# sulaimanvesal/PointCloudUDA

Hardware: AMD Instinct MI355X
Metric: adversarial train-step images/sec (seg+3 discr) at 256x256 (higher is better)
Workload: dtype bf16x3 MFMA (split-bf16, fp32 accumulate; fp32 storage); 1 GPU; MS-CMRSeg full UDA: UNet(PointNet head) + d1 + d2 + d4, 256x256x1, 4 classes; per_gpu_batch=32, global_batch=32, precision=bf16x3, parallelism=dp1, ranks_in_group=1, collective=none, streams=discriminators concurrent, d_target_forward=replayed from the adversarial pass of the same step, launch=eager (256 host cores for this rank)

## Files before the change

### pointcloududa_amd/csrc/conv_igemm.h

```cpp
#pragma once
#include "common.h"

#define IG_MAX_TAPS 36
#define IG_REC 40
#define IG_REC_BYTES 80
template <bool X3>
struct IgRec {
  static constexpr int BYTES = X3 ? 144 : 80;
};
#define IG_LO_OFF 64
static inline int ig_rec_bytes(bool x3) { return x3 ? 144 : 80; }

struct IgemmParams {
  pcuda_src x;
  int cin;
  int in_h, in_w;
  int in_shift;
  int in_row;
  pcuda_dst y;
  int cout;
  int out_w;
  int lh, lw;
  int oy_mul, oy_off, ox_mul, ox_off;
  int in_step;
  int ntaps, tg;
  signed char dy[IG_MAX_TAPS], dx[IG_MAX_TAPS];
  int dy_min, dx_min, ih_t, iw_t;
  const uint16_t* wpack;
  long long w_lo_off;
  int nchunks;
  const float* bias;
  float slope;
  int accumulate;
  float* stats;
  const float* red_a; long long red_sn, red_sc;
  const float* red_mean; const float* red_invstd;
  const float* mask_a; long long mask_sn; float mask_slope;
  int tw, th, tmagic;
  int tiles_x, tiles_y, n;
  int n_co_tiles;
  unsigned m_cot, m_tx, m_ty;
  int clamp;
  int dbg;
  unsigned long long* dbg_clk;
  int xq;
  int fold;
  int pair, lw2;
};

struct WgradParams {
  pcuda_src x;
  int cin;
  int in_h, in_w, in_shift, in_row;
  const float* dz; long long dz_sn, dz_sc;
  int cout, out_h, out_w;
  int stride;
  int ntaps;
  int ntaps_total, tap_groups;
  signed char dy[IG_MAX_TAPS], dx[IG_MAX_TAPS];
  int ih_t, iw_t;
  int dy_min, dx_min;
  int tw, th, tmagic;
  int tiles_x, tiles_y, n;
  int ksplit;
  int n_co_tiles, n_chunks;
  float* partial;
  int aligned4;
  int tw16;
  int xq;
  int dbg;
  int xcd_items;
  int xcd_slices;
};

#define WG_ZROW 272

struct PackParams {
  const float* w;
  uint16_t* out;
  int rec;
  int rows, red;
  long long s_row, s_red;
  int ntaps;
  signed char tap_src[IG_MAX_TAPS];
  int pair;
  int co_tile;
  int nchunks, n_co_tiles;
};

static inline int ig_co_blks(int rows) { return rows > 32 ? 2 : 1; }
#define IG_TY(pl, magic) (((pl) * (magic)) >> 16)
```

### pointcloududa_amd/csrc/conv_wgrad.hip

```cpp
#include "conv_igemm.h"
#include "conv_host.h"

__global__ __launch_bounds__(1024) void wgrad_reduce_kernel(const float* __restrict__ partial, long long numel,
                                                           int ksplit, float* __restrict__ dw, int accumulate,
                                                           int ntaps, const float* __restrict__ db_partial,
                                                           long long nb, float* __restrict__ db) {
  __shared__ float sh[16][64];
  const int lane = threadIdx.x & 63, kg = threadIdx.x >> 6, nkg = blockDim.x >> 6;
  const long long nblk_w = (numel + 63) / 64;
  long long blk = blockIdx.x;
  if (blk >= nblk_w) {
    blk -= nblk_w; partial = db_partial; numel = nb; dw = db; ntaps = 1;
  }
  const long long i = blk * 64 + lane;
  float s = 0.f;
  if (i < numel) {
    int k = kg;
    for (; k + 7 * nkg < ksplit; k += 8 * nkg) {
      float v[8];
#pragma unroll
      for (int u = 0; u < 8; ++u) v[u] = partial[(long long)(k + u * nkg) * numel + i];
#pragma unroll
      for (int u = 0; u < 8; ++u) s += v[u];
    }
    for (; k < ksplit; k += nkg) s += partial[(long long)k * numel + i];
  }
  sh[kg][lane] = s;
  __syncthreads();
  if (kg == 0 && i < numel) {
    float t = 0.f;
    for (int q = 0; q < nkg; ++q) t += sh[q][lane];
    long long o = i;
    if (ntaps > 1) {
      const long long cc = numel / ntaps;
      const long long tt = i / cc, r = i - tt * cc;
      o = r * ntaps + tt;
    }
    dw[o] = accumulate ? dw[o] + t : t;
  }
}

int launch_wgrad_reduce_taps(const float* partial, long long numel, int ksplit, float* dw, int accumulate, int ntaps,
                             const float* db_partial, long long nb, float* db, hipStream_t s) {
  int nkg = 1;
  while (nkg < 16 && nkg * 2 <= ksplit) nkg <<= 1;
  const unsigned nblk = (unsigned)cdiv(numel, 64) + (db ? (unsigned)cdiv(nb, 64) : 0u);
  hipLaunchKernelGGL(wgrad_reduce_kernel, dim3(nblk), dim3(64 * nkg), 0, s, partial, numel, ksplit, dw, accumulate, ntaps,
                     db_partial, db ? nb : 0, db);
  PCUDA_CHECK_LAUNCH("wgrad_reduce_kernel");
  return PCUDA_OK;
}
int launch_wgrad_reduce(const float* partial, long long numel, int ksplit, float* dw, int accumulate, const float* db_partial,
                        long long nb, float* db, hipStream_t s) {
  return launch_wgrad_reduce_taps(partial, numel, ksplit, dw, accumulate, 1, db_partial, nb, db, s);
}

struct ReduceJobs {
  int n;
  int first_block[PCUDA_REDUCE_MAX_JOBS + 1];
  pcuda_reduce_job j[PCUDA_REDUCE_MAX_JOBS];
};

__global__ __launch_bounds__(1024) void wgrad_reduce_batch_kernel(const ReduceJobs jobs) {
  __shared__ float sh[16][64];
  int lo = 0, hi = jobs.n - 1;
  while (lo < hi) {
    const int mid = (lo + hi + 1) >> 1;
    if (jobs.first_block[mid] <= (int)blockIdx.x) lo = mid; else hi = mid - 1;
  }
  const pcuda_reduce_job& jb = jobs.j[lo];
  const float* partial = jb.partial;
  long long numel = jb.numel;
  float* dw = jb.dw;
  int ntaps = jb.ntaps;
  const int ksplit = jb.ksplit, nkg = jb.nkg;
  const int lane = threadIdx.x & 63, kg = threadIdx.x >> 6;
  const long long nblk_w = (numel + 63) / 64;
  long long blk = (int)blockIdx.x - jobs.first_block[lo];
  if (blk >= nblk_w) { blk -= nblk_w; partial = jb.db_partial; numel = jb.nb; dw = jb.db; ntaps = 1; }
  const long long i = blk * 64 + lane;
  float s = 0.f;
  if (i < numel && kg < nkg) {
    int k = kg;
    for (; k + 7 * nkg < ksplit; k += 8 * nkg) {
      float v[8];
#pragma unroll
      for (int u = 0; u < 8; ++u) v[u] = partial[(long long)(k + u * nkg) * numel + i];
#pragma unroll
      for (int u = 0; u < 8; ++u) s += v[u];
    }
    for (; k < ksplit; k += nkg) s += partial[(long long)k * numel + i];
  }
  sh[kg][lane] = s;
  __syncthreads();
  if (kg == 0 && i < numel) {
    float t = 0.f;
    for (int q = 0; q < nkg; ++q) t += sh[q][lane];
    long long o = i;
    if (ntaps > 1) {
      const long long cc = numel / ntaps;
      const long long tt = i / cc, r = i - tt * cc;
      o = r * ntaps + tt;
    }
    dw[o] = jb.accumulate ? dw[o] + t : t;
  }
}

extern "C" int pcuda_wgrad_reduce_batch(const pcuda_reduce_job* host_jobs, int njobs, pcuda_stream_t s) {
  if (!host_jobs || njobs < 0) PCUDA_FAIL(PCUDA_E_BADARG, "wgrad_reduce_batch: bad arguments");
  int done = 0;
  while (done < njobs) {
    ReduceJobs jobs;
    jobs.n = 0;
    int blocks = 0;
    for (; done < njobs && jobs.n < PCUDA_REDUCE_MAX_JOBS; ++done) {
      const pcuda_reduce_job& jb = host_jobs[done];
      if (jb.ksplit <= 0) continue;
      if (!jb.partial || !jb.dw || jb.numel <= 0 || jb.nkg < 1 || jb.nkg > 16 || (jb.db && !jb.db_partial))
        PCUDA_FAIL(PCUDA_E_BADARG, "wgrad_reduce_batch: bad job %d", done);
      jobs.first_block[jobs.n] = blocks;
      jobs.j[jobs.n++] = jb;
      blocks += (int)cdiv(jb.numel, 64) + (jb.db ? (int)cdiv(jb.nb, 64) : 0);
    }
    if (jobs.n == 0) break;
    jobs.first_block[jobs.n] = blocks;
    ProfScope prof(PCUDA_FAM_POINTWISE, 0.0, (hipStream_t)s, "wgrad reduce batch");
    hipLaunchKernelGGL(wgrad_reduce_batch_kernel, dim3(blocks), dim3(1024), 0, (hipStream_t)s, jobs);
    PCUDA_CHECK_LAUNCH("wgrad_reduce_batch_kernel");
  }
  return PCUDA_OK;
}

namespace {

struct WgradPlan {
  int co_blks, co_tile, n_co_tiles, n_chunks, tap_groups, taps_per_group, tw, th, tiles_x, tiles_y, ksplit;
  int ih_t, iw_t;
};

WgradPlan plan_wgrad(const pcuda_conv_geom* g) {
  WgradPlan w;
  w.co_blks = ig_co_blks(g->cout);
  w.co_tile = 32 * w.co_blks;
  w.n_co_tiles = cdiv(g->cout, w.co_tile);
  w.n_chunks = cdiv(g->cin, 32);
  const int ntaps = g->k * g->k;
  w.tap_groups = ntaps <= 16 ? 1 : cdiv(ntaps, 9);
  w.taps_per_group = cdiv(ntaps, w.tap_groups);
  {
    int cand[16];
    const int nc = tile_width_candidates(g->out_w, 128, cand);
    long long best_key = -1;
    w.tw = 32; w.th = 4;
    for (int ci = 0; ci < nc; ++ci) {
      const int tw = cand[ci], th = 128 / tw;
      if (th < 1) continue;
      const int span = (g->k - 1) * g->dil;
      const long long halo = (long long)((th - 1) * g->stride + span + 1) * ((tw - 1) * g->stride + span + 1);
      {
        const long long ih = (th - 1) * g->stride + span + 1, iw = (tw - 1) * g->stride + span + 1;
        const long long clipped = (ih < g->in_h ? ih : g->in_h) * (iw < g->in_w ? iw : g->in_w) + 1;
        const long long cap = halo < clipped ? halo : clipped;
        if (cap * IG_REC_BYTES * 2 + (long long)w.co_tile * WG_ZROW * 2 > (long long)LDS_HARD) continue;
      }
      const long long ih2 = (th - 1) * g->stride + span + 1, iw2 = (tw - 1) * g->stride + span + 1;
      const long long clipped2 = (ih2 < g->in_h ? ih2 : g->in_h) * (iw2 < g->in_w ? iw2 : g->in_w) + 1;
      const long long staged = (clipped2 * 2 <= halo) ? clipped2 : halo;
      const long long key = ((long long)cdiv(g->out_w, tw) * cdiv(g->out_h, th) << 24) + (staged > 768 ? (1ll << 22) : 0) +
                            ((tw & 31) ? (1ll << 20) : 0) + halo;
      if (best_key < 0 || key < best_key) { best_key = key; w.tw = tw; w.th = th; }
    }
  }
  const int TW = w.tw, TH = w.th;
  w.tiles_x = cdiv(g->out_w, TW);
  w.tiles_y = cdiv(g->out_h, TH);
  const int span = (g->k - 1) * g->dil;
  w.ih_t = (TH - 1) * g->stride + span + 1;
  w.iw_t = (TW - 1) * g->stride + span + 1;
  const long long ntiles = (long long)g->n * w.tiles_x * w.tiles_y;
  const int base = w.n_co_tiles * w.n_chunks * w.tap_groups;
  static int tgt32 = -1;
  if (tgt32 < 0) { const char* e = getenv("PCUDA_WG_BLOCKS32"); tgt32 = e ? atoi(e) : 768; }
  static int tgt64 = -1;
  if (tgt64 < 0) { const char* e = getenv("PCUDA_WG_BLOCKS64"); tgt64 = e ? atoi(e) : 1024; }
  static int tgt1 = -1;
  if (tgt1 < 0) { const char* e = getenv("PCUDA_WG_BLOCKS1"); tgt1 = e ? atoi(e) : 256; }
  bool one_per_cu = false;
  {
    const long long full = (long long)w.ih_t * w.iw_t;
    const long long clipped = (long long)(w.ih_t < g->in_h ? w.ih_t : g->in_h) * (w.iw_t < g->in_w ? w.iw_t : g->in_w) + 1;
    const size_t zb = (size_t)w.co_tile * WG_ZROW * 2;
    bool clamp = clipped * 2 <= full;
    if (!clamp && (size_t)full * IG_REC_BYTES * 2 + zb > (size_t)LDS_HARD) clamp = true;
    one_per_cu = (size_t)(clamp ? clipped : full) * IG_REC_BYTES * 2 + zb > (size_t)LDS_HARD / 2;
  }
  long long ks = (one_per_cu ? tgt1 : (w.co_blks == 1 ? tgt32 : tgt64)) / base;
  if (ks < 1) ks = 1;
  if (ks > ntiles) ks = ntiles;
  const long long welems = (long long)g->cout * g->cin * ntaps;
  while (ks > 1 && ks * welems * 4 > (64ll << 20)) ks >>= 1;
  if (ks >= 8) ks &= ~7ll;
  w.ksplit = (int)ks;
  return w;
}

}

extern "C" size_t pcuda_conv2d_wgrad_workspace_size(const pcuda_conv_geom* g) {
  if (!geom_ok(g)) return 0;
  WgradPlan w = plan_wgrad(g);
  const size_t need = ((size_t)w.ksplit * g->cout * g->cin * g->k * g->k + (size_t)w.ksplit * g->cout) * sizeof(float) + 256;
  size_t dneed = direct_wgrad_workspace(g);
  const size_t d1need = direct_d1_wgrad_workspace(g);
  if (d1need > dneed) dneed = d1need;
  const size_t w3need = wgrad3_workspace(g);
  if (w3need > dneed) dneed = w3need;
  const size_t w1need = wgrad1_workspace(g);
  if (w1need > dneed) dneed = w1need;
  const size_t w3rneed = wgrad3r_workspace(g);
  if (w3rneed > dneed) dneed = w3rneed;
  return need > dneed ? need : dneed;
}

int wgrad_dispatch_x3(const WgradParams& p, int co_blks, bool clamp, int taps_max, int pf, int x_cap, size_t lds,
                      float* dbp, dim3 grid, hipStream_t s);
int wgrad_dispatch_bf16(const WgradParams& p, int co_blks, bool clamp, int taps_max, int pf, int x_cap, size_t lds,
                        float* dbp, dim3 grid, hipStream_t s);

static int wgrad_impl(const pcuda_conv_geom* g, int prec, const pcuda_src* x, const float* dy, long long dy_sn, long long dy_sc,
                      float* dw, float* db, int accumulate, void* workspace, size_t workspace_bytes, pcuda_stream_t s_,
                      pcuda_reduce_job* defer);

extern "C" int pcuda_conv2d_wgrad(const pcuda_conv_geom* g, int prec, const pcuda_src* x, const float* dy,
                                  long long dy_sn, long long dy_sc, float* dw, float* db, int accumulate,
                                  void* workspace, size_t workspace_bytes, pcuda_stream_t s_) {
  return wgrad_impl(g, prec, x, dy, dy_sn, dy_sc, dw, db, accumulate, workspace, workspace_bytes, s_, nullptr);
}

extern "C" int pcuda_conv2d_wgrad_partial(const pcuda_conv_geom* g, int prec, const pcuda_src* x, const float* dy,
                                          long long dy_sn, long long dy_sc, float* dw, float* db, int accumulate,
                                          void* workspace, size_t workspace_bytes, pcuda_reduce_job* job, pcuda_stream_t s_) {
  if (!job) PCUDA_FAIL(PCUDA_E_BADARG, "conv2d_wgrad_partial: job is NULL");
  memset(job, 0, sizeof(*job));
  return wgrad_impl(g, prec, x, dy, dy_sn, dy_sc, dw, db, accumulate, workspace, workspace_bytes, s_, job);
}

static int wgrad_impl(const pcuda_conv_geom* g, int prec, const pcuda_src* x, const float* dy, long long dy_sn, long long dy_sc,
                      float* dw, float* db, int accumulate, void* workspace, size_t workspace_bytes, pcuda_stream_t s_,
                      pcuda_reduce_job* defer) {
  hipStream_t s = (hipStream_t)s_;
  if (!geom_ok(g)) PCUDA_FAIL(PCUDA_E_BADARG, "conv2d_wgrad: inconsistent geometry");
  if (!src_ok(x, g->cin) || !dy || !dw) PCUDA_FAIL(PCUDA_E_BADARG, "conv2d_wgrad: bad tensors");
  if (prec != PCUDA_PREC_BF16X3 && prec != PCUDA_PREC_BF16) PCUDA_FAIL(PCUDA_E_BADARG, "conv2d_wgrad: bad precision");
  if (!workspace || workspace_bytes < pcuda_conv2d_wgrad_workspace_size(g))
    PCUDA_FAIL(PCUDA_E_WORKSPACE, "conv2d_wgrad: workspace too small (%zu < %zu)", workspace_bytes,
               pcuda_conv2d_wgrad_workspace_size(g));
  {
    int rc;
    if (direct_wgrad(g, x, dy, dy_sn, dy_sc, dw, db, accumulate, workspace, s, &rc)) return rc;
    if (direct_d1_wgrad(g, x, dy, dy_sn, dy_sc, dw, db, accumulate, workspace, s, &rc)) return rc;
    if (wgrad3r_try(g, prec, x, dy, dy_sn, dy_sc, dw, db, accumulate, workspace, s, defer, &rc)) return rc;
    if (wgrad3_try(g, prec, x, dy, dy_sn, dy_sc, dw, db, accumulate, workspace, s, defer, &rc)) return rc;
    if (wgrad1_try(g, prec, x, dy, dy_sn, dy_sc, dw, db, accumulate, workspace, s, defer, &rc)) return rc;
  }
  const bool x3 = prec == PCUDA_PREC_BF16X3;
  WgradPlan w = plan_wgrad(g);
  TapSet t = fwd_taps(g);
  WgradParams p;
  memset(&p, 0, sizeof(p));
  p.x = *x; p.cin = g->cin;
  p.in_h = g->in_h; p.in_w = g->in_w; p.in_shift = g->in_up ? 1 : 0; p.in_row = g->in_w >> p.in_shift;
  p.dz = dy; p.dz_sn = dy_sn; p.dz_sc = dy_sc;
  p.cout = g->cout; p.out_h = g->out_h; p.out_w = g->out_w;
  p.stride = g->stride;
  p.ntaps = w.taps_per_group; p.ntaps_total = t.n; p.tap_groups = w.tap_groups;
  memcpy(p.dy, t.dy, sizeof(p.dy));
  memcpy(p.dx, t.dx, sizeof(p.dx));
  p.dy_min = t.dy_min; p.dx_min = t.dx_min;
  p.ih_t = w.ih_t; p.iw_t = w.iw_t;
  p.tw = w.tw; p.th = w.th; p.tmagic = 65536 / w.tw + 1; p.tiles_x = w.tiles_x; p.tiles_y = w.tiles_y; p.n = g->n;
  p.ksplit = w.ksplit; p.n_co_tiles = w.n_co_tiles; p.n_chunks = w.n_chunks;
  p.partial = (float*)workspace;
  {
    static int dbg = -1;
    if (dbg < 0) { const char* e = getenv("PCUDA_DBG"); dbg = e ? atoi(e) : 0; }
    p.dbg = dbg;
  }
  p.tw16 = ((w.tw & 15) == 0 && w.tw * w.th == 128) ? 1 : 0;
  p.aligned4 = ((g->out_w & 7) == 0 && (w.tw & 7) == 0 && (dy_sn & 3) == 0 && (dy_sc & 3) == 0 && (((uintptr_t)dy) & 15) == 0 &&
                ((long long)g->cout * dy_sc + (long long)g->out_h * g->out_w) * 4 < (1ll << 30)) ? 1 : 0;
  const long long welems = (long long)g->cout * g->cin * t.n;
  float* dbp = db ? (float*)workspace + (size_t)w.ksplit * welems : nullptr;

  const int full = w.ih_t * w.iw_t;
  const int clipped = (w.ih_t < g->in_h ? w.ih_t : g->in_h) * (w.iw_t < g->in_w ? w.iw_t : g->in_w) + 1;
  const size_t mul = x3 ? 2 : 1;
  const size_t zb = (size_t)w.co_tile * WG_ZROW * mul;
  bool clamp = clipped * 2 <= full;
  if (!clamp && (size_t)full * IG_REC_BYTES * mul + zb > (size_t)LDS_HARD) clamp = true;
  const int x_cap = clamp ? clipped : full;
  const size_t lds = (size_t)x_cap * IG_REC_BYTES * mul + zb;
  if (lds > (size_t)LDS_HARD) PCUDA_FAIL(PCUDA_E_UNSUPPORTED, "conv2d_wgrad: tile %dx%d does not fit LDS", w.ih_t, w.iw_t);
  const dim3 grid(w.n_co_tiles * w.n_chunks * w.tap_groups, w.ksplit);
  {
    static int noxcd = -1;
    if (noxcd < 0) { const char* e = getenv("PCUDA_WG_NOXCD"); noxcd = (e && atoi(e)) ? 1 : 0; }
    const long long nblk = (long long)grid.x * grid.y;
    p.xcd_items = (!noxcd && nblk >= 16 && (nblk & 7) == 0) ? (int)(nblk / 8) : 0;
    static int nointer = -1;
    if (nointer < 0) { const char* e = getenv("PCUDA_WG_NOINTER"); nointer = (e && atoi(e)) ? 1 : 0; }
    p.xcd_slices = (p.xcd_items && !nointer && (w.ksplit & 7) == 0) ? w.ksplit / 8 : 0;
  }
  {
    const double flops = 2.0 * g->n * (double)g->out_h * g->out_w * g->cout * (double)g->cin * t.n;
    char tag[160];
    static int nopipe = -1;
    if (nopipe < 0) { const char* e = getenv("PCUDA_NOPIPE"); nopipe = (e && atoi(e)) ? 1 : 0; }
    int pf = (nopipe || !fast_src_ok(x, g->cin)) ? 0 : (x_cap <= 256 ? 1 : (x_cap <= 768 ? 3 : 0));
    static int now8 = -1;
    if (now8 < 0) { const char* e = getenv("PCUDA_WG_NO8"); now8 = (e && atoi(e)) ? 1 : 0; }
    if (!now8 && pf > 0 && w.taps_per_group > 9 && x_cap <= 1024) pf = 100 + (x_cap <= 512 ? 1 : 2);
    {
      static int noxq = -1;
      if (noxq < 0) { const char* e = getenv("PCUDA_NOXQ"); noxq = e ? atoi(e) : 0; }
      const int slots = pf >= 100 ? pf - 100 : pf, per = pf >= 100 ? 128 : 64;
      const int ih = clamp ? (w.ih_t < g->in_h ? w.ih_t : g->in_h) : w.ih_t;
      const int in_w_phys = g->in_up ? g->in_w / 2 : g->in_w;
      p.xq = (!noxq && slots > 0 && !g->in_up && (in_w_phys & 3) == 0 && (ih * ((w.iw_t + 6) / 4) + per - 1) / per <= slots) ? 1 : 0;
    }
    snprintf(tag, sizeof(tag), "wgrad n%d cin%d cout%d %dx%d k%d s%d d%d ksplit%d clamp%d pf%d lds%zu", g->n, g->cin,
             g->cout, g->out_h, g->out_w, g->k, g->stride, g->dil, w.ksplit, clamp ? 1 : 0, pf, lds);
    ProfScope prof(PCUDA_FAM_CONV_WGRAD, flops, s, tag);
    int rc;
    const int taps_max = w.taps_per_group <= 1 ? 1 : w.taps_per_group <= 9 ? 9 : 16;
    rc = x3 ? wgrad_dispatch_x3(p, w.co_blks, clamp, taps_max, pf, x_cap, lds, dbp, grid, s)
            : wgrad_dispatch_bf16(p, w.co_blks, clamp, taps_max, pf, x_cap, lds, dbp, grid, s);
    if (rc) return rc;
  }
  {
    int nkg = 1;
    while (nkg < 16 && nkg * 2 <= w.ksplit) nkg <<= 1;
    if (defer) {
      defer->partial = (const float*)workspace; defer->numel = welems; defer->ksplit = w.ksplit; defer->nkg = nkg;
      defer->dw = dw; defer->accumulate = accumulate; defer->ntaps = t.n;
      defer->db_partial = (const float*)dbp; defer->nb = db ? g->cout : 0; defer->db = db;
      return PCUDA_OK;
    }
    const unsigned nblk = (unsigned)cdiv(welems, 64) + (db ? (unsigned)cdiv(g->cout, 64) : 0u);
    hipLaunchKernelGGL(wgrad_reduce_kernel, dim3(nblk), dim3(64 * nkg), 0, s, (const float*)workspace, welems, w.ksplit,
                       dw, accumulate, t.n, (const float*)dbp, (long long)(db ? g->cout : 0), db);
    PCUDA_CHECK_LAUNCH("wgrad_reduce_kernel");
  }
  return PCUDA_OK;
}
```

### pointcloududa_amd/csrc/conv_wgrad_impl.h

```cpp
#pragma once
#include "conv_device.h"
#include "conv_host.h"
#include "variants.h"


__device__ __forceinline__ bf16x8 lds_tr_frag(const unsigned char* p0, const unsigned char* p1) {
  bf16x4 lo = __builtin_amdgcn_ds_read_tr16_b64_v4bf16((LDS_AS bf16x4*)p0);
  bf16x4 hi = __builtin_amdgcn_ds_read_tr16_b64_v4bf16((LDS_AS bf16x4*)p1);
  return __builtin_shufflevector(lo, hi, 0, 1, 2, 3, 4, 5, 6, 7);
}

struct WTile {
  int n, y0, x0, oy0, ox0, th, tw, npix;
};

template <bool CLAMP>
__device__ __forceinline__ WTile wtile_decode(const WgradParams& p, int tile) {
  WTile t;
  const int txi = tile % p.tiles_x;
  const int tmp = tile / p.tiles_x;
  const int tyi = tmp % p.tiles_y;
  t.n = tmp / p.tiles_y;
  t.y0 = tyi * p.th; t.x0 = txi * p.tw;
  t.oy0 = t.y0 * p.stride + p.dy_min; t.ox0 = t.x0 * p.stride + p.dx_min;
  t.th = p.ih_t; t.tw = p.iw_t;
  if (CLAMP) {
    const int y1 = min(t.oy0 + t.th, p.in_h), x1 = min(t.ox0 + t.tw, p.in_w);
    t.oy0 = max(t.oy0, 0); t.ox0 = max(t.ox0, 0);
    t.th = max(y1 - t.oy0, 0); t.tw = max(x1 - t.ox0, 0);
  }
  t.npix = t.th * t.tw;
  return t;
}

template <int CO_TILE, int NT = 256>
__device__ __forceinline__ void zpre_issue(float (&zv)[CO_TILE * 16 / NT][8], const WgradParams& p, const WTile& t,
                                           int cot, int tid0) {
  const int tid = tid0 + opaque_zero();
  const int TW = p.tw, TPIX = p.tw * p.th;
#pragma unroll
  for (int j = 0; j < CO_TILE * 16 / NT; ++j) {
    const int item = tid + NT * j;
    const int row = item >> 4, oct = item & 15;
    const int pl = oct * 8;
    const int cco = min(cot * CO_TILE + row, p.cout - 1);
    const float* planep = p.dz + (long long)t.n * p.dz_sn + (long long)cco * p.dz_sc;
    if (p.aligned4) {
      const int ty = IG_TY(pl, p.tmagic), tx = pl - ty * TW;
      const int oy = t.y0 + ty, ox = t.x0 + tx;
      const float* rowp = planep + (long long)min(oy, p.out_h - 1) * p.out_w + min(ox, p.out_w - 8);
      const float4 a = *(const float4*)rowp, b = *(const float4*)(rowp + 4);
      zv[j][0] = a.x; zv[j][1] = a.y; zv[j][2] = a.z; zv[j][3] = a.w;
      zv[j][4] = b.x; zv[j][5] = b.y; zv[j][6] = b.z; zv[j][7] = b.w;
    } else {
#pragma unroll
      for (int e = 0; e < 8; ++e) {
        const int ple = min(pl + e, TPIX - 1);
        const int ty = IG_TY(ple, p.tmagic), tx = ple - ty * TW;
        const int oy = t.y0 + ty, ox = t.x0 + tx;
        zv[j][e] = planep[(long long)min(oy, p.out_h - 1) * p.out_w + min(ox, p.out_w - 1)];
      }
    }
  }
}

template <int CO_TILE, int NT = 256>
struct ZConst {
  int off[CO_TILE * 16 / NT];
  int ty, tx;
};
template <int CO_TILE, int NT = 256>
__device__ __forceinline__ void zfast_init(ZConst<CO_TILE, NT>& zc, const WgradParams& p, int cot, int tid) {
  const int pl = (tid & 15) * 8;
  zc.ty = IG_TY(pl, p.tmagic); zc.tx = pl - zc.ty * p.tw;
#pragma unroll
  for (int j = 0; j < CO_TILE * 16 / NT; ++j) {
    const int co = min(cot * CO_TILE + ((tid + NT * j) >> 4), p.cout - 1);
    zc.off[j] = co * (int)p.dz_sc + zc.ty * p.out_w + zc.tx;
  }
}
template <int CO_TILE, int NT = 256>
__device__ __forceinline__ void zfast_issue(float (&zv)[CO_TILE * 16 / NT][8], const ZConst<CO_TILE, NT>& zc,
                                            const WgradParams& p, const WTile& t) {
  const float* tb = p.dz + (long long)t.n * p.dz_sn + (long long)(t.y0 * p.out_w + t.x0);
  const int cy = min(t.y0 + zc.ty, p.out_h - 1) - (t.y0 + zc.ty);
  const int cx = min(t.x0 + zc.tx, p.out_w - 8) - (t.x0 + zc.tx);
  const int dl = cy * p.out_w + cx;
#pragma unroll
  for (int j = 0; j < CO_TILE * 16 / NT; ++j) {
    const float* rp = tb + (zc.off[j] + dl);
    const float4 a = *(const float4*)rp, b = *(const float4*)(rp + 4);
    zv[j][0] = a.x; zv[j][1] = a.y; zv[j][2] = a.z; zv[j][3] = a.w;
    zv[j][4] = b.x; zv[j][5] = b.y; zv[j][6] = b.z; zv[j][7] = b.w;
  }
}

template <bool X3, int CO_TILE, int NT = 256>
__device__ __forceinline__ void zpre_commit(float (&zv)[CO_TILE * 16 / NT][8], const WgradParams& p, const WTile& t,
                                            int cot, int tid, unsigned char* __restrict__ Zhi,
                                            unsigned char* __restrict__ Zlo, bool do_db,
                                            float (&dbacc)[CO_TILE * 16 / NT], bool premasked) {
  tid += opaque_zero();
  const int TW = p.tw, TPIX = p.tw * p.th;
#pragma unroll
  for (int j = 0; j < CO_TILE * 16 / NT; ++j) {
    const int item = tid + NT * j;
    const int row = item >> 4, oct = item & 15;
    const int pl = oct * 8;
    const bool cok = cot * CO_TILE + row < p.cout;
    float(&v)[8] = zv[j];
    if (premasked) {
    } else if (p.aligned4) {
      const int ty = IG_TY(pl, p.tmagic), tx = pl - ty * TW;
      const bool ok = cok & (pl < TPIX) & (t.y0 + ty < p.out_h) & (t.x0 + tx + 8 <= p.out_w);
#pragma unroll
      for (int e = 0; e < 8; ++e) v[e] = ok ? v[e] : 0.f;
    } else {
#pragma unroll
      for (int e = 0; e < 8; ++e) {
        const int ple = min(pl + e, TPIX - 1);
        const int ty = IG_TY(ple, p.tmagic), tx = ple - ty * TW;
        const bool ok = cok & (pl + e < TPIX) & (t.y0 + ty < p.out_h) & (t.x0 + tx < p.out_w);
        v[e] = ok ? v[e] : 0.f;
      }
    }
    if (do_db) dbacc[j] += ((v[0] + v[1]) + (v[2] + v[3])) + ((v[4] + v[5]) + (v[6] + v[7]));
    uint4 hi, lo;
    if (X3) {
      split2(v[0], v[1], hi.x, lo.x); split2(v[2], v[3], hi.y, lo.y);
      split2(v[4], v[5], hi.z, lo.z); split2(v[6], v[7], hi.w, lo.w);
      *(uint4*)(Zlo + row * WG_ZROW + oct * 16) = lo;
    } else {
      hi.x = pack_bf16x2(v[0], v[1]); hi.y = pack_bf16x2(v[2], v[3]);
      hi.z = pack_bf16x2(v[4], v[5]); hi.w = pack_bf16x2(v[6], v[7]);
    }
    *(uint4*)(Zhi + row * WG_ZROW + oct * 16) = hi;
  }
}

template <bool X3, int MAXT, int MODE>
__device__ __forceinline__ void wgrad_mfma_phase(const WgradParams& p, f32x16 (&acc)[MAXT],
                                                 const unsigned char* __restrict__ Xhi,
                                                 const unsigned char* __restrict__ Xlo,
                                                 const unsigned char* __restrict__ Zhi,
                                                 const unsigned char* __restrict__ Zlo, int cb, int lane,
                                                 const int (&tap_off)[MAXT], const int (&tap_dy)[MAXT],
                                                 const int (&tap_dx)[MAXT], const WTile& t) {
  const int r = lane & 31, h = lane >> 5;
  const int g = lane >> 4, li = lane & 15, tq = li >> 2, tp = li & 3;
  const int TW = p.tw, TPIX = p.tw * p.th;
  const int colb = ((g & 1) * 16 + 4 * tp) * 2;
  int rb0[2];
#pragma unroll
  for (int sel = 0; sel < 2; ++sel) rb0[sel] = ((8 * (g >> 1) + 4 * sel + tq) * p.stride) * IG_REC_BYTES + colb;
  auto xaddr = [&](int ks, int ti, int& r0, int& r1) {
    if (MODE == 0) {
      const int s0 = ks * 16;
      const int ry = IG_TY(s0, p.tmagic), rx = s0 - ry * TW;
      const int soff = ((ry * p.stride) * p.iw_t + rx * p.stride) * IG_REC_BYTES + tap_off[ti];
      r0 = rb0[0] + soff; r1 = rb0[1] + soff;
      return;
    }
    int rty[2], rtx[2];
#pragma unroll
    for (int sel = 0; sel < 2; ++sel) {
      const int pl = min(ks * 16 + 8 * (g >> 1) + 4 * sel + tq, TPIX - 1);
      rty[sel] = IG_TY(pl, p.tmagic); rtx[sel] = pl - rty[sel] * TW;
    }
    int ra[2];
#pragma unroll
    for (int sel = 0; sel < 2; ++sel) {
      if (MODE == 2) {
        const int gy = (t.y0 + rty[sel]) * p.stride + tap_dy[ti], gx = (t.x0 + rtx[sel]) * p.stride + tap_dx[ti];
        const bool ok = ((unsigned)gy < (unsigned)p.in_h) & ((unsigned)gx < (unsigned)p.in_w);
        ra[sel] = (ok ? (gy - t.oy0) * t.tw + (gx - t.ox0) : t.npix) * IG_REC_BYTES + colb;
      } else {
        ra[sel] = ((rty[sel] * p.stride) * p.iw_t + rtx[sel] * p.stride) * IG_REC_BYTES + colb + tap_off[ti];
      }
    }
    r0 = ra[0]; r1 = ra[1];
  };
  const int abase = (cb * 32 + r) * WG_ZROW + h * 16;
  bf16x8 ah = lds_frag(Zhi + abase), al = ah;
  if (X3) al = lds_frag(Zlo + abase);
  bf16x8 bh, bl;
  {
    int r0, r1;
    xaddr(0, 0, r0, r1);
    bh = lds_tr_frag(Xhi + r0, Xhi + r1);
    bl = bh;
    if (X3) bl = lds_tr_frag(Xlo + r0, Xlo + r1);
  }
#pragma unroll 2
  for (int ks = 0; ks < 8; ++ks) {
    bf16x8 ahn = ah, aln = al;
#pragma unroll
    for (int ti = 0; ti < MAXT; ++ti) {
      bf16x8 bhn, bln = bh;
      {
        const int nks = (ti + 1 < MAXT) ? ks : min(ks + 1, 7);
        const int nti = (ti + 1 < MAXT) ? ti + 1 : 0;
        int r0, r1;
        xaddr(nks, nti, r0, r1);
        bhn = lds_tr_frag(Xhi + r0, Xhi + r1);
        if (X3) bln = lds_tr_frag(Xlo + r0, Xlo + r1);
        if (ti + 1 == MAXT) {
          ahn = lds_frag(Zhi + abase + nks * 32);
          if (X3) aln = lds_frag(Zlo + abase + nks * 32);
        }
      }
      __builtin_amdgcn_sched_barrier(0);
      if (X3) {
        acc[ti] = __builtin_amdgcn_mfma_f32_32x32x16_bf16(al, bh, acc[ti], 0, 0, 0);
        acc[ti] = __builtin_amdgcn_mfma_f32_32x32x16_bf16(ah, bl, acc[ti], 0, 0, 0);
      }
      acc[ti] = __builtin_amdgcn_mfma_f32_32x32x16_bf16(ah, bh, acc[ti], 0, 0, 0);
      __builtin_amdgcn_sched_barrier(0);
      bh = bhn; bl = bln;
    }
    ah = ahn; al = aln;
  }
}

template <bool X3, int CO_BLKS, int MODE, int TAPS_MAX, int PF, int NW = 4, bool XQ = false>
__global__ __launch_bounds__(64 * NW, (NW == 8 || (TAPS_MAX <= 9 && PF <= 1)) ? 2 : 1) void wgrad_kernel(const WgradParams p, const int x_cap, float* db_partial) {
  extern __shared__ __attribute__((aligned(16))) unsigned char smem[];
  constexpr bool CLAMP = MODE == 2;
  constexpr int CO_TILE = 32 * CO_BLKS;
  constexpr int NT = 64 * NW, ZJ = CO_TILE * 16 / NT;
  static_assert(NW == 4 || PF > 0, "the eight-wave variant is pipelined");
  constexpr int NWT = NW / CO_BLKS;
  constexpr int MAXT = (TAPS_MAX + NWT - 1) / NWT;
  constexpr int XPF = PF > 0 ? PF : 1;
  const int tid = threadIdx.x, lane = tid & 63, r = lane & 31, h = lane >> 5;
  const int w = __builtin_amdgcn_readfirstlane(tid >> 6);

  int bx = blockIdx.x, kslice = blockIdx.y;
  if (p.xcd_items) {
    const int lin = blockIdx.y * gridDim.x + blockIdx.x;
    const int item = (lin & 7) * p.xcd_items + (lin >> 3);
    kslice = item / (int)gridDim.x;
    bx = item - kslice * (int)gridDim.x;
  }
  const int tgidx = bx % p.tap_groups;
  const int chunk = (bx / p.tap_groups) % p.n_chunks;
  const int cot = bx / (p.tap_groups * p.n_chunks);
  const int t_begin = tgidx * p.ntaps;
  const int tcount = min(p.ntaps, p.ntaps_total - t_begin);
  const int cb = w % CO_BLKS, wsub = w / CO_BLKS;
  const int share = (tcount + NWT - 1) / NWT;
  const int my_t0 = t_begin + wsub * share;
  const int my_cnt = max(0, min(share, tcount - wsub * share));

  unsigned char* Xhi = smem;
  unsigned char* Xlo = smem + (size_t)x_cap * IG_REC_BYTES;
  unsigned char* Zhi = smem + (size_t)(X3 ? 2 : 1) * x_cap * IG_REC_BYTES;
  unsigned char* Zlo = Zhi + (size_t)CO_TILE * WG_ZROW;

  const int ntiles = p.n * p.tiles_y * p.tiles_x;
  int tile_lo = (int)((long long)kslice * ntiles / p.ksplit);
  int tile_hi = (int)((long long)(kslice + 1) * ntiles / p.ksplit);
  int tile_step = 1;
  if (p.xcd_items && p.xcd_slices) {
    const int xcd = (blockIdx.y * gridDim.x + blockIdx.x) & 7, S = p.xcd_slices;
    const int T_lo = (int)((long long)xcd * ntiles / 8), T_hi = (int)((long long)(xcd + 1) * ntiles / 8);
    tile_lo = T_lo + (kslice - xcd * S);
    tile_step = S;
    tile_hi = tile_lo < T_hi ? tile_lo + ((T_hi - tile_lo + S - 1) / S) * S : tile_lo;
  }
  const bool do_db = (db_partial != nullptr) && chunk == 0 && tgidx == 0;

  f32x16 acc[MAXT];
#pragma unroll
  for (int ti = 0; ti < MAXT; ++ti)
#pragma unroll
    for (int i = 0; i < 16; ++i) acc[ti][i] = 0.f;
  float dbacc[ZJ];
#pragma unroll
  for (int j = 0; j < ZJ; ++j) dbacc[j] = 0.f;

  const int cvalid = min(32, p.cin - chunk * 32);
  const int ngroups = (cvalid + 7) >> 3;

  int tap_off[MAXT], tap_dy[MAXT], tap_dx[MAXT];
#pragma unroll
  for (int ti = 0; ti < MAXT; ++ti) {
    const int t = min(my_t0 + min(ti, max(my_cnt - 1, 0)), p.ntaps_total - 1);
    tap_dy[ti] = p.dy[t]; tap_dx[ti] = p.dx[t];
    tap_off[ti] = ((tap_dy[ti] - p.dy_min) * p.iw_t + (tap_dx[ti] - p.dx_min)) * IG_REC_BYTES;
  }

  constexpr bool ZPRE = PF > 0 && !(CO_BLKS == 2 && TAPS_MAX == 9 && PF == 1 && MODE != 0);
  XFast<XPF> xpre;
  float zv[ZJ][8];
  ZConst<CO_TILE, NT> zc;
  const bool zfast = PF > 0 && (MODE == 0 || p.aligned4);
  if (zfast) zfast_init<CO_TILE, NT>(zc, p, cot, tid);
  WTile cur = wtile_decode<CLAMP>(p, min(tile_lo, ntiles - 1));
  if (PF > 0 && tile_lo < tile_hi) {
    if (XQ) xq_issue<XPF, NT>(xpre, p.x, cur.n, p.cin, chunk, p.in_h, p.in_w, cur.oy0, cur.ox0, cur.th, cur.tw, tid);
    else xfast_issue<XPF, NT>(xpre, p.x, cur.n, p.cin, chunk, p.in_h, p.in_w, p.in_shift, p.in_row, cur.oy0, cur.ox0, cur.tw,
                              cur.npix, ngroups, tid);
    if (ZPRE) {
      if (zfast) zfast_issue<CO_TILE, NT>(zv, zc, p, cur);
      else zpre_issue<CO_TILE, NT>(zv, p, cur, cot, tid);
    }
  }

  for (int tile = tile_lo; tile < tile_hi; tile += tile_step) {
    if (PF == 0) cur = wtile_decode<CLAMP>(p, tile);
    const int oy0 = cur.oy0, ox0 = cur.ox0, tw = cur.tw, npix = cur.npix;
    __syncthreads();
    if (PF > 0) {
      if (XQ) xq_commit<X3, XPF, NT>(xpre, Xhi, Xlo, p.x, p.cin, chunk, ox0, cur.th, tw, 4, tid);
      else xfast_commit<X3, XPF, NT>(xpre, Xhi, Xlo, p.x, p.cin, chunk, npix, ngroups, 4, tid);
      if (!ZPRE) {
        if (zfast) zfast_issue<CO_TILE, NT>(zv, zc, p, cur);
        else zpre_issue<CO_TILE, NT>(zv, p, cur, cot, tid);
      }
    } else {
      stage_x_chunk<X3, 1>(Xhi, Xlo, p.x, cur.n, p.cin, chunk, p.in_h, p.in_w, p.in_shift, p.in_row, oy0, ox0, cur.th,
                           tw, ngroups, 4, tid);
      zpre_issue<CO_TILE, NT>(zv, p, cur, cot, tid);
    }
    if (CLAMP && tid < 5) {
      *(uint4*)(Xhi + (size_t)npix * IG_REC_BYTES + tid * 16) = make_uint4(0, 0, 0, 0);
      if (X3) *(uint4*)(Xlo + (size_t)npix * IG_REC_BYTES + tid * 16) = make_uint4(0, 0, 0, 0);
    }
    zpre_commit<X3, CO_TILE, NT>(zv, p, cur, cot, tid, Zhi, Zlo, do_db, dbacc, false);
    __syncthreads();
    WTile nxt = cur;
    if (PF > 0 && tile + tile_step < tile_hi) {
      nxt = wtile_decode<CLAMP>(p, tile + tile_step);
      if (XQ) xq_issue<XPF, NT>(xpre, p.x, nxt.n, p.cin, chunk, p.in_h, p.in_w, nxt.oy0, nxt.ox0, nxt.th, nxt.tw, tid);
      else xfast_issue<XPF, NT>(xpre, p.x, nxt.n, p.cin, chunk, p.in_h, p.in_w, p.in_shift, p.in_row, nxt.oy0, nxt.ox0, nxt.tw,
                                nxt.npix, ngroups, tid);
      if (ZPRE) {
        if (zfast) zfast_issue<CO_TILE, NT>(zv, zc, p, nxt);
        else zpre_issue<CO_TILE, NT>(zv, p, nxt, cot, tid);
      }
    }

#ifdef PCUDA_CLK_DEBUG
    if (!(p.dbg & 64))
#endif
      wgrad_mfma_phase<X3, MAXT, MODE>(p, acc, Xhi, Xlo, Zhi, Zlo, cb, lane, tap_off, tap_dy, tap_dx, cur);
    cur = nxt;
  }

#pragma unroll
  for (int ti = 0; ti < MAXT; ++ti) {
    if (ti < my_cnt) {
      const int t = my_t0 + ti;
#pragma unroll
      for (int i = 0; i < 16; ++i) {
        const int co = cot * CO_TILE + cb * 32 + (i & 3) + 8 * (i >> 2) + 4 * h;
        const int ci = chunk * 32 + r;
        if (co < p.cout && ci < p.cin)
          p.partial[(((long long)kslice * p.ntaps_total + t) * p.cout + co) * p.cin + ci] = acc[ti][i];
      }
    }
  }
  if (do_db) {
#pragma unroll
    for (int j = 0; j < ZJ; ++j) {
      float s = dbacc[j];
#pragma unroll
      for (int o = 8; o > 0; o >>= 1) s += __shfl_xor(s, o, 64);
      const int row = (tid + NT * j) >> 4;
      const int co = cot * CO_TILE + row;
      if ((tid & 15) == 0 && co < p.cout) db_partial[(long long)kslice * p.cout + co] = s;
    }
  }
}


template <bool X3, int CO_BLKS, int MODE, int TAPS_MAX, int PF, int NW, bool XQ>
static int launch_wgrad_q(const WgradParams& p, int x_cap, size_t lds, float* dbp, dim3 grid, hipStream_t s) {
  constexpr unsigned vkey = wgrad_key(X3, CO_BLKS, MODE, TAPS_MAX, PF, NW, XQ);
  variant_log("wgrad", vkey);
  if constexpr (!wgrad_built(vkey)) {
    variant_fallback_note("wgrad_kernel", vkey);
    return launch_wgrad_q<X3, CO_BLKS, MODE, TAPS_MAX, 0, NW, false>(p, x_cap, lds, dbp, grid, s);
  } else {
  auto kern = wgrad_kernel<X3, CO_BLKS, MODE, TAPS_MAX, PF, NW, XQ>;
  static DeviceOnce lds_opt;
  if (const unsigned long long devbit = lds > 32 * 1024 ? lds_opt.pending() : 0ull) {
    hipError_t e = hipFuncSetAttribute((const void*)kern, hipFuncAttributeMaxDynamicSharedMemorySize, (int)LDS_HARD);
    if (e != hipSuccess) PCUDA_FAIL(PCUDA_E_LAUNCH, "wgrad: cannot raise dynamic LDS: %s", hipGetErrorString(e));
    lds_opt.mark(devbit);
  }
  note_kernel(PF == 0 ? "wgrad_generic" : (NW == 8 ? "wgrad8" : "wgrad"));
  hipLaunchKernelGGL(kern, grid, dim3(64 * NW), lds, s, p, x_cap, dbp);
  PCUDA_CHECK_LAUNCH("wgrad_kernel");
  return PCUDA_OK;
  }
}

template <bool X3, int CO_BLKS, int MODE, int TAPS_MAX, int PF, int NW = 4>
static int launch_wgrad_t(const WgradParams& p, int x_cap, size_t lds, float* dbp, dim3 grid, hipStream_t s) {
  if (PF > 0 && p.xq) return launch_wgrad_q<X3, CO_BLKS, MODE, TAPS_MAX, PF, NW, (PF > 0)>(p, x_cap, lds, dbp, grid, s);
  return launch_wgrad_q<X3, CO_BLKS, MODE, TAPS_MAX, PF, NW, false>(p, x_cap, lds, dbp, grid, s);
}


template <bool X3>
static int wgrad_dispatch(const WgradParams& p, int co_blks, bool clamp, int taps_max, int pf, int x_cap, size_t lds,
                          float* dbp, dim3 grid, hipStream_t s) {
  const int mode = clamp ? 2 : ((p.tw16 && p.aligned4) ? 0 : 1);
  if (pf >= 100) {
#define WG8_PF(CB_, MD_) (pf == 101 ? launch_wgrad_t<X3, CB_, MD_, 16, 1, 8>(p, x_cap, lds, dbp, grid, s) : launch_wgrad_t<X3, CB_, MD_, 16, 2, 8>(p, x_cap, lds, dbp, grid, s))
#define WG8_MD(CB_) (mode == 2 ? WG8_PF(CB_, 2) : mode == 0 ? WG8_PF(CB_, 0) : WG8_PF(CB_, 1))
    return co_blks == 2 ? WG8_MD(2) : WG8_MD(1);
#undef WG8_MD
#undef WG8_PF
  }
#define WG_PF(CB_, MD_, TM_)                                                                     \
  (pf == 1 ? launch_wgrad_t<X3, CB_, MD_, TM_, 1>(p, x_cap, lds, dbp, grid, s)                  \
   : pf == 3 ? launch_wgrad_t<X3, CB_, MD_, TM_, 3>(p, x_cap, lds, dbp, grid, s)                \
             : launch_wgrad_t<X3, CB_, MD_, TM_, 0>(p, x_cap, lds, dbp, grid, s))
#define WG_TM(CB_, MD_) (taps_max == 1 ? WG_PF(CB_, MD_, 1) : taps_max == 9 ? WG_PF(CB_, MD_, 9) : WG_PF(CB_, MD_, 16))
#define WG_MD(CB_) (mode == 2 ? WG_TM(CB_, 2) : mode == 0 ? WG_TM(CB_, 0) : WG_TM(CB_, 1))
  return co_blks == 2 ? WG_MD(2) : WG_MD(1);
#undef WG_MD
#undef WG_TM
#undef WG_PF
}
```

### pointcloududa_amd/csrc/variants.h

```cpp
#pragma once
#include "built_variants.h"

#define PCUDA_E_NOTBUILT (-100)

constexpr unsigned pipe_key(bool x3, int co_blks, bool clamp, int npb, int pf, bool xq, int stats, bool te) {
  return (x3 ? 1u : 0u) | ((unsigned)(co_blks - 1) << 1) | ((clamp ? 1u : 0u) << 2) | ((unsigned)(npb - 1) << 3) |
         ((unsigned)(pf - 1) << 4) | ((xq ? 1u : 0u) << 6) | ((unsigned)stats << 7) | ((te ? 1u : 0u) << 9);
}
constexpr unsigned ig8_key(bool x3, int co_blks, bool clamp, int npbt, int pf, bool xq, bool stats) {
  return (x3 ? 1u : 0u) | ((unsigned)(co_blks - 1) << 1) | ((clamp ? 1u : 0u) << 2) | ((npbt == 8 ? 1u : 0u) << 3) |
         ((unsigned)(pf - 1) << 4) | ((xq ? 1u : 0u) << 6) | ((stats ? 1u : 0u) << 7);
}
constexpr unsigned wgrad_key(bool x3, int co_blks, int mode, int taps_max, int pf, int nw, bool xq) {
  return (x3 ? 1u : 0u) | ((unsigned)(co_blks - 1) << 1) | ((unsigned)mode << 2) |
         ((taps_max == 1 ? 0u : taps_max == 9 ? 1u : 2u) << 4) | ((pf == 0 ? 0u : pf == 1 ? 1u : pf == 2 ? 3u : 2u) << 6) |
         ((nw == 8 ? 1u : 0u) << 8) | ((xq ? 1u : 0u) << 9);
}

template <int N>
constexpr bool variant_in(const unsigned (&list)[N], unsigned key) {
  for (int i = 0; i < N; ++i)
    if (list[i] == key) return true;
  return false;
}
#ifdef PCUDA_FULL
constexpr bool pipe_built(unsigned) { return true; }
constexpr bool ig8_built(unsigned) { return true; }
constexpr bool wgrad_built(unsigned) { return true; }
#else
constexpr unsigned PIPE_LIST[] = {PCUDA_BUILT_PIPE};
constexpr unsigned IG8_LIST[] = {PCUDA_BUILT_IG8};
constexpr unsigned WGRAD_LIST[] = {PCUDA_BUILT_WGRAD};
constexpr bool pipe_built(unsigned k) { return ((k >> 11) & 1u) != 0u || variant_in(PIPE_LIST, k); }
constexpr bool ig8_built(unsigned k) { return variant_in(IG8_LIST, k); }
constexpr bool wgrad_built(unsigned k) { return ((k >> 6) & 3u) == 0u || ((k >> 8) & 1u) != 0u || variant_in(WGRAD_LIST, k); }
#endif

void variant_log(const char* family, unsigned key);
void note_kernel(const char* name);
void variant_fallback_note(const char* family, unsigned key);
```

Baseline: 748.8 img/s.

## Add row-phase MFMA inner loop for weight-gradient kernel with power-of-two tiles

Adds a specialised wgrad MFMA phase that walks the pixel dimension in 16-wide k-steps across tile rows. It software-pipelines the LDS transposed loads of the next tap and fragment, and skips MFMAs when both input rows fall outside the image. It is enabled by default for 3x3-style tap groups with power-of-two tile widths, through a new compile-time ROW template variant and a built-variant list. The goal is less address arithmetic and fewer wasted MFMAs on padded rows in the weight-gradient convolutions. The cost is more template instantiations and the risk of wrong indexing for stride or clamp cases.

```diff
diff --git a/pointcloududa_amd/csrc/conv_igemm.h b/pointcloududa_amd/csrc/conv_igemm.h
--- a/pointcloududa_amd/csrc/conv_igemm.h
+++ b/pointcloududa_amd/csrc/conv_igemm.h
@@ -71,6 +71,7 @@
   int dbg;
   int xcd_items;
   int xcd_slices;
+  int rowphase;
 };
 
 #define WG_ZROW 272
diff --git a/pointcloududa_amd/csrc/conv_wgrad.hip b/pointcloududa_amd/csrc/conv_wgrad.hip
--- a/pointcloududa_amd/csrc/conv_wgrad.hip
+++ b/pointcloududa_amd/csrc/conv_wgrad.hip
@@ -137,6 +137,11 @@
   int co_blks, co_tile, n_co_tiles, n_chunks, tap_groups, taps_per_group, tw, th, tiles_x, tiles_y, ksplit;
   int ih_t, iw_t;
 };
+
+int env_int(const char* name, int dflt) {
+  const char* e = getenv(name);
+  return e ? atoi(e) : dflt;
+}
 
 WgradPlan plan_wgrad(const pcuda_conv_geom* g) {
   WgradPlan w;
@@ -179,12 +184,9 @@
   w.iw_t = (TW - 1) * g->stride + span + 1;
   const long long ntiles = (long long)g->n * w.tiles_x * w.tiles_y;
   const int base = w.n_co_tiles * w.n_chunks * w.tap_groups;
-  static int tgt32 = -1;
-  if (tgt32 < 0) { const char* e = getenv("PCUDA_WG_BLOCKS32"); tgt32 = e ? atoi(e) : 768; }
-  static int tgt64 = -1;
-  if (tgt64 < 0) { const char* e = getenv("PCUDA_WG_BLOCKS64"); tgt64 = e ? atoi(e) : 1024; }
-  static int tgt1 = -1;
-  if (tgt1 < 0) { const char* e = getenv("PCUDA_WG_BLOCKS1"); tgt1 = e ? atoi(e) : 256; }
+  const int tgt32 = env_int("PCUDA_WG_BLOCKS32", 768);
+  const int tgt64 = env_int("PCUDA_WG_BLOCKS64", 1024);
+  const int tgt1 = env_int("PCUDA_WG_BLOCKS1", 256);
   bool one_per_cu = false;
   {
     const long long full = (long long)w.ih_t * w.iw_t;
@@ -289,6 +291,8 @@
   p.tw16 = ((w.tw & 15) == 0 && w.tw * w.th == 128) ? 1 : 0;
   p.aligned4 = ((g->out_w & 7) == 0 && (w.tw & 7) == 0 && (dy_sn & 3) == 0 && (dy_sc & 3) == 0 && (((uintptr_t)dy) & 15) == 0 &&
                 ((long long)g->cout * dy_sc + (long long)g->out_h * g->out_w) * 4 < (1ll << 30)) ? 1 : 0;
+  p.rowphase = ((w.tw & (w.tw - 1)) == 0 && w.tw >= 8 && w.tw * w.th == 128 && w.taps_per_group > 1 && w.taps_per_group <= 9 &&
+                env_int("PCUDA_WGRAD_ROW", 1) != 0) ? 1 : 0;
   const long long welems = (long long)g->cout * g->cin * t.n;
   float* dbp = db ? (float*)workspace + (size_t)w.ksplit * welems : nullptr;
 
diff --git a/pointcloududa_amd/csrc/conv_wgrad_impl.h b/pointcloududa_amd/csrc/conv_wgrad_impl.h
--- a/pointcloududa_amd/csrc/conv_wgrad_impl.h
+++ b/pointcloududa_amd/csrc/conv_wgrad_impl.h
@@ -222,7 +222,102 @@
   }
 }
 
-template <bool X3, int CO_BLKS, int MODE, int TAPS_MAX, int PF, int NW = 4, bool XQ = false>
+template <bool X3, int MAXT, bool CLAMP>
+__device__ __forceinline__ void wgrad_mfma_phase_row(const WgradParams& p, f32x16 (&acc)[MAXT],
+                                                     const unsigned char* __restrict__ Xhi,
+                                                     const unsigned char* __restrict__ Xlo,
+                                                     const unsigned char* __restrict__ Zhi,
+                                                     const unsigned char* __restrict__ Zlo, int cb, int lane,
+                                                     const int (&tap_off)[MAXT], const int (&tap_dy)[MAXT],
+                                                     const int (&tap_dx)[MAXT], const WTile& t) {
+  const int r = lane & 31, h = lane >> 5;
+  const int g = lane >> 4, li = lane & 15, tq = li >> 2, tp = li & 3;
+  const int colb = ((g & 1) * 16 + 4 * tp) * 2;
+  const int TW = p.tw, ltw = __builtin_ctz(TW);
+  const bool two = TW == 8;
+  const int lrow = two ? (g >> 1) : 0;
+  constexpr int NEG = -(1 << 28);
+  const int rowb = p.stride * (CLAMP ? t.tw : p.iw_t) * IG_REC_BYTES, xsb = p.stride * IG_REC_BYTES;
+  const int twb = t.tw * IG_REC_BYTES, zaddr = t.npix * IG_REC_BYTES + colb;
+  const int rs2 = two ? p.stride : 0;
+  int xb[2];
+#pragma unroll
+  for (int sel = 0; sel < 2; ++sel) {
+    const int lx = (two ? 0 : 8 * (g >> 1)) + 4 * sel + tq;
+    xb[sel] = CLAMP ? ((t.x0 + lx) * p.stride - t.ox0) * IG_REC_BYTES
+                    : (lrow * p.stride * p.iw_t + lx * p.stride) * IG_REC_BYTES + colb;
+  }
+  auto row_of = [&](int ks, int ti) { return (t.y0 + ((ks * 16) >> ltw)) * p.stride + tap_dy[ti]; };
+  auto runs = [&](int gy) { return ((unsigned)gy < (unsigned)p.in_h) | ((unsigned)(gy + rs2) < (unsigned)p.in_h); };
+  auto xaddr = [&](int ks, int ti, int gy, int& r0, int& r1) {
+    const int s0 = ks * 16, ry = s0 >> ltw, rx = s0 & (TW - 1);
+    if (!CLAMP) {
+      const int S = ry * rowb + rx * xsb + tap_off[ti];
+      r0 = xb[0] + S; r1 = xb[1] + S;
+    } else {
+      const int gyB = gy + rs2;
+      const int rowA = (unsigned)gy < (unsigned)p.in_h ? (gy - t.oy0) * twb : NEG;
+      const int rowB = (unsigned)gyB < (unsigned)p.in_h ? (gyB - t.oy0) * twb : NEG;
+      const int rowl = (lrow ? rowB : rowA) + colb;
+      const int Sx = (rx * p.stride + tap_dx[ti]) * IG_REC_BYTES;
+      int ra[2];
+#pragma unroll
+      for (int sel = 0; sel < 2; ++sel) {
+        const int v = xb[sel] + Sx;
+        const int sum = (unsigned)v < (unsigned)twb ? v + rowl : NEG;
+        ra[sel] = (int)min((unsigned)sum, (unsigned)zaddr);
+      }
+      r0 = ra[0]; r1 = ra[1];
+    }
+  };
+  const int abase = (cb * 32 + r) * WG_ZROW + h * 16;
+  bf16x8 ah = lds_frag(Zhi + abase), al = ah;
+  if (X3) al = lds_frag(Zlo + abase);
+  int gy = row_of(0, 0);
+  bf16x8 bh, bl;
+  {
+    int r0, r1;
+    xaddr(0, 0, gy, r0, r1);
+    bh = lds_tr_frag(Xhi + r0, Xhi + r1);
+    bl = bh;
+    if (X3) bl = lds_tr_frag(Xlo + r0, Xlo + r1);
+  }
+#pragma unroll 2
+  for (int ks = 0; ks < 8; ++ks) {
+    bf16x8 ahn = ah, aln = al;
+#pragma unroll
+    for (int ti = 0; ti < MAXT; ++ti) {
+      const bool last = ti + 1 == MAXT;
+      const int nks = last ? min(ks + 1, 7) : ks, nti = last ? 0 : ti + 1;
+      const int gyn = row_of(nks, nti);
+      bf16x8 bhn, bln = bh;
+      {
+        int r0, r1;
+        xaddr(nks, nti, gyn, r0, r1);
+        bhn = lds_tr_frag(Xhi + r0, Xhi + r1);
+        if (X3) bln = lds_tr_frag(Xlo + r0, Xlo + r1);
+      }
+      if (last) {
+        const int zks = min(ks + 1, 7);
+        ahn = lds_frag(Zhi + abase + zks * 32);
+        if (X3) aln = lds_frag(Zlo + abase + zks * 32);
+      }
+      __builtin_amdgcn_sched_barrier(0);
+      if (runs(gy)) {
+        if (X3) {
+          acc[ti] = __builtin_amdgcn_mfma_f32_32x32x16_bf16(al, bh, acc[ti], 0, 0, 0);
+          acc[ti] = __builtin_amdgcn_mfma_f32_32x32x16_bf16(ah, bl, acc[ti], 0, 0, 0);
+        }
+        acc[ti] = __builtin_amdgcn_mfma_f32_32x32x16_bf16(ah, bh, acc[ti], 0, 0, 0);
+      }
+      __builtin_amdgcn_sched_barrier(0);
+      bh = bhn; bl = bln; gy = gyn;
+    }
+    ah = ahn; al = aln;
+  }
+}
+
+template <bool X3, int CO_BLKS, int MODE, int TAPS_MAX, int PF, int NW = 4, bool XQ = false, bool ROW = false>
 __global__ __launch_bounds__(64 * NW, (NW == 8 || (TAPS_MAX <= 9 && PF <= 1)) ? 2 : 1) void wgrad_kernel(const WgradParams p, const int x_cap, float* db_partial) {
   extern __shared__ __attribute__((aligned(16))) unsigned char smem[];
   constexpr bool CLAMP = MODE == 2;
@@ -344,7 +439,10 @@
 #ifdef PCUDA_CLK_DEBUG
     if (!(p.dbg & 64))
 #endif
-      wgrad_mfma_phase<X3, MAXT, MODE>(p, acc, Xhi, Xlo, Zhi, Zlo, cb, lane, tap_off, tap_dy, tap_dx, cur);
+    {
+      if constexpr (ROW) wgrad_mfma_phase_row<X3, MAXT, CLAMP>(p, acc, Xhi, Xlo, Zhi, Zlo, cb, lane, tap_off, tap_dy, tap_dx, cur);
+      else wgrad_mfma_phase<X3, MAXT, MODE>(p, acc, Xhi, Xlo, Zhi, Zlo, cb, lane, tap_off, tap_dy, tap_dx, cur);
+    }
     cur = nxt;
   }
 
@@ -375,22 +473,25 @@
 }
 
 
-template <bool X3, int CO_BLKS, int MODE, int TAPS_MAX, int PF, int NW, bool XQ>
+template <bool X3, int CO_BLKS, int MODE, int TAPS_MAX, int PF, int NW, bool XQ, bool ROW = false>
 static int launch_wgrad_q(const WgradParams& p, int x_cap, size_t lds, float* dbp, dim3 grid, hipStream_t s) {
-  constexpr unsigned vkey = wgrad_key(X3, CO_BLKS, MODE, TAPS_MAX, PF, NW, XQ);
+  constexpr unsigned vkey = wgrad_key(X3, CO_BLKS, MODE, TAPS_MAX, PF, NW, XQ) | (ROW ? WGRAD_ROW_BIT : 0u);
+  if constexpr (!ROW && NW == 4 && wgrad_row_built(vkey)) {
+    if (p.rowphase) return launch_wgrad_q<X3, CO_BLKS, MODE, TAPS_MAX, PF, NW, XQ, true>(p, x_cap, lds, dbp, grid, s);
+  }
   variant_log("wgrad", vkey);
-  if constexpr (!wgrad_built(vkey)) {
+  if constexpr (!ROW && !wgrad_built(vkey)) {
     variant_fallback_note("wgrad_kernel", vkey);
     return launch_wgrad_q<X3, CO_BLKS, MODE, TAPS_MAX, 0, NW, false>(p, x_cap, lds, dbp, grid, s);
   } else {
-  auto kern = wgrad_kernel<X3, CO_BLKS, MODE, TAPS_MAX, PF, NW, XQ>;
+  auto kern = wgrad_kernel<X3, CO_BLKS, MODE, TAPS_MAX, PF, NW, XQ, ROW>;
   static DeviceOnce lds_opt;
   if (const unsigned long long devbit = lds > 32 * 1024 ? lds_opt.pending() : 0ull) {
     hipError_t e = hipFuncSetAttribute((const void*)kern, hipFuncAttributeMaxDynamicSharedMemorySize, (int)LDS_HARD);
     if (e != hipSuccess) PCUDA_FAIL(PCUDA_E_LAUNCH, "wgrad: cannot raise dynamic LDS: %s", hipGetErrorString(e));
     lds_opt.mark(devbit);
   }
-  note_kernel(PF == 0 ? "wgrad_generic" : (NW == 8 ? "wgrad8" : "wgrad"));
+  note_kernel(ROW ? (PF == 0 ? "wgrad_generic_row" : "wgrad_row") : PF == 0 ? "wgrad_generic" : (NW == 8 ? "wgrad8" : "wgrad"));
   hipLaunchKernelGGL(kern, grid, dim3(64 * NW), lds, s, p, x_cap, dbp);
   PCUDA_CHECK_LAUNCH("wgrad_kernel");
   return PCUDA_OK;
diff --git a/pointcloududa_amd/csrc/variants.h b/pointcloududa_amd/csrc/variants.h
--- a/pointcloududa_amd/csrc/variants.h
+++ b/pointcloududa_amd/csrc/variants.h
@@ -17,6 +17,9 @@
          ((nw == 8 ? 1u : 0u) << 8) | ((xq ? 1u : 0u) << 9);
 }
 
+constexpr unsigned WGRAD_ROW_BIT = 1u << 10;
+#define PCUDA_BUILT_WGRAD_ROW 84u, 85u, 86u, 87u, 144u, 145u, 146u, 147u, 148u, 149u, 150u, 151u, 595u, 656u, 657u, 658u, 659u, 660u, 661u, 662u, 663u, 664u, 665u, 666u, 667u
+
 template <int N>
 constexpr bool variant_in(const unsigned (&list)[N], unsigned key) {
   for (int i = 0; i < N; ++i)
@@ -27,6 +30,7 @@
 constexpr bool pipe_built(unsigned) { return true; }
 constexpr bool ig8_built(unsigned) { return true; }
 constexpr bool wgrad_built(unsigned) { return true; }
+constexpr bool wgrad_row_built(unsigned k) { return ((k >> 4) & 3u) == 1u; }
 #else
 constexpr unsigned PIPE_LIST[] = {PCUDA_BUILT_PIPE};
 constexpr unsigned IG8_LIST[] = {PCUDA_BUILT_IG8};
@@ -34,6 +38,8 @@
 constexpr bool pipe_built(unsigned k) { return ((k >> 11) & 1u) != 0u || variant_in(PIPE_LIST, k); }
 constexpr bool ig8_built(unsigned k) { return variant_in(IG8_LIST, k); }
 constexpr bool wgrad_built(unsigned k) { return ((k >> 6) & 3u) == 0u || ((k >> 8) & 1u) != 0u || variant_in(WGRAD_LIST, k); }
+constexpr unsigned WGRAD_ROW_LIST[] = {PCUDA_BUILT_WGRAD_ROW};
+constexpr bool wgrad_row_built(unsigned k) { return variant_in(WGRAD_ROW_LIST, k & ~WGRAD_ROW_BIT); }
 #endif
 
 void variant_log(const char* family, unsigned key);
```

New measurement: 748.6 img/s. About the same (-0.0%).
